# PaddlePaddle/Paddle

Hardware: AMD Instinct MI355X
Metric: tokens/sec (whole node) GPT-3-6.7B Fleet sharding-3 (higher is better)
Workload: dtype bf16; 1 GPU; model=gpt3-6.7b, global_batch=12, seq_len=2048, parallelism=sharding3_dp1

## Files before the change

### csrc/kernels/fa_bwd.hip

```cpp
#include "fa_common.h"

namespace pa {

template <int D>
__global__ void fa_bwd_delta_kernel(const short* __restrict__ dog, const short* __restrict__ og,
                                    float* __restrict__ delta, int H, int Sq,
                                    long long rows,
                                    long long do_sb, long long do_sh, long long do_ss,
                                    long long o_sb, long long o_sh, long long o_ss) {
  constexpr int LPR = D / 8, RPP = 256 / LPR, UNR = 4;
  const int sub = threadIdx.x % LPR;
  const int rin = threadIdx.x / LPR;
  const bool h_fast = do_sh < do_ss;
  for (long long r0 = (long long)blockIdx.x * (RPP * UNR); r0 < rows;
       r0 += (long long)gridDim.x * (RPP * UNR)) {
    shortx8 a[UNR], bb[UNR];
    long long di[UNR];
#pragma unroll
    for (int u = 0; u < UNR; ++u) {
      const long long r = r0 + u * RPP + rin;
      di[u] = -1;
      if (r < rows) {
        int sq, h, b;
        if (h_fast) {
// ... 200 lines not shown
      constexpr int elems = QB * D;
      for (int flat = tid * 8; flat < elems; flat += NT * 8) {
        int row = flat / D, col = flat % D;
        shortx8 qv, dv;
        if (q0 + row < Sq) {
          qv = *reinterpret_cast<const shortx8*>(qg + qbase + (long long)(q0 + row) * q_ss + col);
          dv = *reinterpret_cast<const shortx8*>(dog + dobase + (long long)(q0 + row) * do_ss + col);
        } else {
          for (int i = 0; i < 8; ++i) { qv[i] = 0; dv[i] = 0; }
        }
        const unsigned o = dkv_off<D>(row, col >> 3);
        *reinterpret_cast<shortx8*>(qbuf + o) = qv;
        *reinterpret_cast<shortx8*>(qbuf + TILE + o) = dv;
      }
    }
  };
  auto load_stats = [&](int q0, float* lse_o, float* delta_o) {
#pragma unroll
    for (int nt = 0; nt < 4; ++nt) {
      int q_abs = q0 + nt * 16 + l16;
      lse_o[nt] = (q_abs < Sq) ? lseg[lse_base + q_abs] : INFINITY;
      delta_o[nt] = (q_abs < Sq) ? deltag[lse_base + q_abs] : 0.f;
    }
  };

  char* const pw = lds + 4 * TILE + wq * PW;
  const unsigned lds_a = (unsigned)(size_t)(__attribute__((address_space(3))) char*)lds;
  const unsigned tr_q = l16 >> 2, tr_p = l16 & 3;
  unsigned bt_a[NDT];
#pragma unroll
  for (int dt = 0; dt < NDT; ++dt)
    bt_a[dt] = lds_a + dkv_off<D>(8 * lg + tr_q, 2 * dt + (tr_p >> 1)) + ((tr_p & 1) << 3);
  const unsigned pa_lo = lds_a + 4 * TILE + wq * PW + dkv_p_off(8 * lg + tr_q, tr_p);
  const unsigned pa_hi = lds_a + 4 * TILE + wq * PW + dkv_p_off(8 * lg + 4 + tr_q, tr_p);
  float lse_n[4], delta_n[4];
  if (q_start < Sq) {
    stage(q_start, lds);
    load_stats(q_start, lse_n, delta_n);
  }
  int cur = 0;
  for (int q0 = q_start; q0 < Sq; q0 += QB) {
    asm volatile("s_waitcnt vmcnt(0)" ::: "memory");
    __syncthreads();
    const unsigned boff = cur * (2 * TILE);
    const char* q_t = lds + boff;
    float lse_v[4], delta_v[4];
#pragma unroll
    for (int nt = 0; nt < 4; ++nt) { lse_v[nt] = lse_n[nt]; delta_v[nt] = delta_n[nt]; }
    if (q0 + QB < Sq) {
      stage(q0 + QB, lds + (cur ^ 1) * (2 * TILE));
      load_stats(q0 + QB, lse_n, delta_n);
    }
    cur ^= 1;
    const char* do_t = q_t + TILE;

    floatx4 pt[4];
    const int kv_abs0 = kv0 + wq * 16 + lg * 4;
#pragma unroll
    for (int nt = 0; nt < 4; ++nt) {
      floatx4 st = {0.f, 0.f, 0.f, 0.f};
#pragma unroll
      for (int kk = 0; kk < NKK; ++kk) {
        shortx8 qfr = *reinterpret_cast<const shortx8*>(
            q_t + dkv_off<D>(nt * 16 + l16, kk * 4 + lg));
        st = mfma_bf16(kf[kk], qfr, st);
      }
      const int q_abs = q0 + nt * 16 + l16;
      const bool bnd = (q0 + QB > Sq) || (kv0 + KVEXT > Skv) ||
                       (CAUSAL && q0 < kv0 + KVEXT);
      if (bnd) {
#pragma unroll
        for (int r = 0; r < 4; ++r) {
          int kv_abs = kv_abs0 + r;
          float p = __expf(st[r] * scale - lse_v[nt]);
          if (q_abs >= Sq || kv_abs >= Skv || (CAUSAL && kv_abs > q_abs)) p = 0.f;
          pt[nt][r] = p;
        }
      } else {
#pragma unroll
        for (int r = 0; r < 4; ++r)
          pt[nt][r] = __expf(st[r] * scale - lse_v[nt]);
      }
    }

    shortx8 pa[2];
    auto put_get = [&]() {
#pragma unroll
      for (int nt = 0; nt < 4; ++nt) {
        shortx4 v = {f2bf(pt[nt][0]), f2bf(pt[nt][1]), f2bf(pt[nt][2]), f2bf(pt[nt][3])};
        *reinterpret_cast<shortx4*>(pw + dkv_p_off(nt * 16 + l16, lg)) = v;
      }
      dkv_tr_read_pa(pa, pa_lo, pa_hi);
    };
    put_get();

    dkv_mma_tr<D, TILE>(dv_acc, pa[0], bt_a, boff);
    dkv_mma_tr<D, TILE + 32 * D * 2>(dv_acc, pa[1], bt_a, boff);

#pragma unroll
    for (int nt = 0; nt < 4; ++nt) {
      floatx4 dp = {0.f, 0.f, 0.f, 0.f};
#pragma unroll
      for (int kk = 0; kk < NKK; ++kk) {
        shortx8 bfr = *reinterpret_cast<const shortx8*>(
            do_t + dkv_off<D>(nt * 16 + l16, kk * 4 + lg));
        dp = mfma_bf16(vf[kk], bfr, dp);
      }
#pragma unroll
      for (int r = 0; r < 4; ++r)
        pt[nt][r] = pt[nt][r] * (dp[r] - delta_v[nt]) * scale;
    }
    put_get();

    dkv_mma_tr<D, 0>(dk_acc, pa[0], bt_a, boff);
    dkv_mma_tr<D, 32 * D * 2>(dk_acc, pa[1], bt_a, boff);
  }

#pragma unroll
  for (int r = 0; r < 4; ++r) {
    int row = kv0 + wq * 16 + lg * 4 + r;
    if (row >= Skv) continue;
#pragma unroll
    for (int dt = 0; dt < NDT; ++dt) {
      dkg[dkbase + (long long)row * dk_ss + dt * 16 + l16] = f2bf(dk_acc[dt][r]);
      dvg[dkbase + (long long)row * dk_ss + dt * 16 + l16] = f2bf(dv_acc[dt][r]);
    }
  }
}

template <int D, bool CAUSAL, bool MASKED, bool DROPOUT, bool VARLEN>
__launch_bounds__(256, 2)
__global__ void fa_bwd_dq32_kernel(const short* __restrict__ dog, const short* __restrict__ qg,
                                   const short* __restrict__ kg, const short* __restrict__ vg,
                                   const float* __restrict__ lseg, const float* __restrict__ deltag,
                                   short* __restrict__ dqg, int B, int H, int Sq, int Skv,
                                   float scale,
                                   long long q_sb, long long q_sh, long long q_ss,
                                   long long k_sb, long long k_sh, long long k_ss,
                                   long long do_sb, long long do_sh, long long do_ss,
                                   long long dq_sb, long long dq_sh, long long dq_ss,
                                   const short* __restrict__ maskg, long long m_sb,
                                   long long m_sh, long long m_sq,
                                   float pdrop, unsigned long long rseed,
                                   unsigned long long roffset,
                                   const int* __restrict__ cu_q,
                                   const int* __restrict__ cu_k,
                                   const int* __restrict__ bmap) {
  constexpr int NW = 4;
  constexpr int NT = NW * 64;
  constexpr int QB = NW * 32;
  constexpr int KB = 64;
  constexpr int NKS = D / 16;
  constexpr int NDT = D / 32;
  constexpr unsigned NAT_RS = D * 2;
  constexpr unsigned KT_RS = KB * 2;
  __shared__ char k_lds[KB * D * 2];
  __shared__ char v_lds[KB * D * 2];
  __shared__ char kt_lds[D * KB * 2];

  const int qblk = blockIdx.y;
  const int bh = blockIdx.x;
  int b = bh / H, h = bh % H;
  int q0, Sq_e = Sq, Skv_e = Skv, cdelta = 0, qglob0 = 0;
  long long qbase, dobase, dqbase, kvbase;
  if (VARLEN) {
    b = 0; h = bh;
    const int seq = bmap[2 * qblk];
    q0 = bmap[2 * qblk + 1];
    const int qs0 = cu_q[seq], ks0 = cu_k[seq];
    Sq_e = cu_q[seq + 1] - qs0;
    Skv_e = cu_k[seq + 1] - ks0;
    cdelta = Skv_e - Sq_e;
    qglob0 = qs0;
    qbase = (long long)qs0 * q_ss + (long long)h * q_sh;
    dobase = (long long)qs0 * do_ss + (long long)h * do_sh;
    dqbase = (long long)qs0 * dq_ss + (long long)h * dq_sh;
    kvbase = (long long)ks0 * k_ss + (long long)h * k_sh;
  } else {
    q0 = (CAUSAL ? ((int)gridDim.y - 1 - qblk) : qblk) * QB;
    qbase = (long long)b * q_sb + (long long)h * q_sh;
    dobase = (long long)b * do_sb + (long long)h * do_sh;
    dqbase = (long long)b * dq_sb + (long long)h * dq_sh;
    kvbase = (long long)b * k_sb + (long long)h * k_sh;
  }
  const long long lse_base = ((long long)bh) * Sq + qglob0;

  const int tid = threadIdx.x;
  const int lane = tid & 63;
  const int wq = tid >> 6;
  const int l32 = lane & 31;
  const int hi = lane >> 5;
  const int q0w = q0 + wq * 32;

  shortx8 qf[NKS], dof[NKS];
  {
    int row = q0w + l32;
    bool ok = row < Sq_e;
#pragma unroll
    for (int ks = 0; ks < NKS; ++ks) {
      if (ok) {
        shortx8 raw = *reinterpret_cast<const shortx8*>(
            qg + qbase + (long long)row * q_ss + ks * 16 + hi * 8);
#pragma unroll
        for (int i = 0; i < 8; ++i) qf[ks][i] = f2bf(bf2f(raw[i]) * scale);
        dof[ks] = *reinterpret_cast<const shortx8*>(
            dog + dobase + (long long)row * do_ss + ks * 16 + hi * 8);
      } else {
        for (int i = 0; i < 8; ++i) { qf[ks][i] = 0; dof[ks][i] = 0; }
      }
    }
  }
  const int q_abs = q0w + l32;
  const float lse_v = (q_abs < Sq_e) ? lseg[lse_base + q_abs] : 1e30f;
  const float delta_v = (q_abs < Sq_e) ? deltag[lse_base + q_abs] : 0.f;

  floatx16 dq_acc[NDT];
#pragma unroll
  for (int dt = 0; dt < NDT; ++dt)
#pragma unroll
    for (int r = 0; r < 16; ++r) dq_acc[dt][r] = 0.f;

  constexpr unsigned KSWZ = (D >= 128) ? 15u : 7u;
  int n_row[KB * D / (NT * 8)], n_colp[KB * D / (NT * 8)];
#pragma unroll
  for (int it = 0; it < KB * D / (NT * 8); ++it) {
    int flat = it * NT * 8 + tid * 8;
    int row = flat / D, col = flat % D;
    n_row[it] = row;
    n_colp[it] = col ^ ((row & (int)KSWZ) << 3);
  }

  const int kv_end = CAUSAL ? min(Skv_e, q0 + QB + cdelta) : Skv_e;
  for (int kv0 = 0; kv0 < kv_end; kv0 += KB) {
    if (kv0 + KB <= Skv_e) {
#pragma unroll
      for (int it = 0; it < KB * D / (NT * 8); ++it) {
        const short* ksrc = kg + kvbase + (long long)(kv0 + n_row[it]) * k_ss + n_colp[it];
        const short* vsrc = vg + kvbase + (long long)(kv0 + n_row[it]) * k_ss + n_colp[it];
        __builtin_amdgcn_global_load_lds(
            (const __attribute__((address_space(1))) unsigned int*)ksrc,
            (__attribute__((address_space(3))) unsigned int*)(k_lds + it * NT * 16 + (tid >> 6) * 64 * 16),
            16, 0, 0);
        __builtin_amdgcn_global_load_lds(
            (const __attribute__((address_space(1))) unsigned int*)vsrc,
            (__attribute__((address_space(3))) unsigned int*)(v_lds + it * NT * 16 + (tid >> 6) * 64 * 16),
            16, 0, 0);
      }
      const int rot = tid & 7;
      for (int flat = tid * 8; flat < KB * D; flat += NT * 8) {
        int row = flat / D, col = flat % D;
        shortx8 kv_ = *reinterpret_cast<const shortx8*>(
            kg + kvbase + (long long)(kv0 + row) * k_ss + col);
#pragma unroll
        for (int j = 0; j < 8; ++j) {
          int i = (j + rot) & 7;
          *reinterpret_cast<short*>(kt_lds + lds_off32(col + i, row * 2, KT_RS)) = kv_[i];
        }
      }
    } else {
      for (int flat = tid * 8; flat < KB * D; flat += NT * 8) {
        int row = flat / D, col = flat % D;
        shortx8 kv_, vv;
        if (kv0 + row < Skv_e) {
          kv_ = *reinterpret_cast<const shortx8*>(kg + kvbase + (long long)(kv0 + row) * k_ss + col);
          vv = *reinterpret_cast<const shortx8*>(vg + kvbase + (long long)(kv0 + row) * k_ss + col);
        } else {
          for (int i = 0; i < 8; ++i) { kv_[i] = 0; vv[i] = 0; }
        }
        *reinterpret_cast<shortx8*>(k_lds + lds_off32w(row, col * 2, NAT_RS, KSWZ)) = kv_;
        *reinterpret_cast<shortx8*>(v_lds + lds_off32w(row, col * 2, NAT_RS, KSWZ)) = vv;
        const int rot = tid & 7;
#pragma unroll
        for (int j = 0; j < 8; ++j) {
          int i = (j + rot) & 7;
          *reinterpret_cast<short*>(kt_lds + lds_off32(col + i, row * 2, KT_RS)) = kv_[i];
        }
      }
    }
    __syncthreads();

    floatx16 st[2], dp[2];
#pragma unroll
    for (int t = 0; t < 2; ++t) {
#pragma unroll
      for (int r = 0; r < 16; ++r) { st[t][r] = 0.f; dp[t][r] = 0.f; }
#pragma unroll
      for (int ks = 0; ks < NKS; ++ks) {
        shortx8 kf = *reinterpret_cast<const shortx8*>(
            k_lds + lds_off32w(t * 32 + l32, (ks * 16 + hi * 8) * 2, NAT_RS, KSWZ));
        st[t] = mfma32_bf16(kf, qf[ks], st[t]);
        shortx8 vf = *reinterpret_cast<const shortx8*>(
            v_lds + lds_off32w(t * 32 + l32, (ks * 16 + hi * 8) * 2, NAT_RS, KSWZ));
        dp[t] = mfma32_bf16(vf, dof[ks], dp[t]);
      }
    }

    if (MASKED && q_abs < Sq_e) {
      const short* mrow = maskg + (long long)b * m_sb + (long long)h * m_sh
                        + (long long)q_abs * m_sq;
#pragma unroll
      for (int t = 0; t < 2; ++t)
#pragma unroll
        for (int g = 0; g < 4; ++g) {
          long long kvb = kv0 + 32 * t + 8 * g + 4 * hi;
          if (kvb + 3 < Skv_e) {
            shortx4 mv = *reinterpret_cast<const shortx4*>(mrow + kvb);
#pragma unroll
            for (int j = 0; j < 4; ++j) st[t][4 * g + j] += bf2f(mv[j]);
          } else {
#pragma unroll
            for (int j = 0; j < 4; ++j)
              if (kvb + j < Skv_e) st[t][4 * g + j] += bf2f(mrow[kvb + j]);
          }
        }
    }
    const bool bnd = (kv0 + KB > Skv_e) || (CAUSAL && kv0 + KB > q_abs + cdelta);
    const float inv_keep = DROPOUT ? 1.f / (1.f - pdrop) : 1.f;
    const unsigned thr24 = DROPOUT ? (unsigned)(pdrop * 16777216.f) : 0u;
    const long long bh_ll = (long long)b * H + h;
#pragma unroll
    for (int t = 0; t < 2; ++t) {
      if (DROPOUT) {
#pragma unroll
        for (int g = 0; g < 4; ++g) {
          long long kvb = kv0 + 32 * t + 8 * g + 4 * hi;
          long long elem = (bh_ll * Sq + (q_abs + qglob0)) * (long long)Skv + kvb;
          uintx4 rv = philox10(rseed, roffset + (unsigned long long)(elem >> 2));
#pragma unroll
          for (int j = 0; j < 4; ++j)
            dp[t][4 * g + j] = ((rv[j] >> 8) >= thr24)
                                   ? dp[t][4 * g + j] * inv_keep : 0.f;
        }
      }
#pragma unroll
      for (int r = 0; r < 16; ++r) {
        float p = __expf(st[t][r] - lse_v);
        if (bnd) {
          int kv_abs = kv0 + 32 * t + (r & 3) + 8 * (r >> 2) + 4 * hi;
          if (kv_abs >= Skv_e || (CAUSAL && kv_abs > q_abs + cdelta)) p = 0.f;
        }
        st[t][r] = p * (dp[t][r] - delta_v) * scale;
      }
    }

#pragma unroll
    for (int ks = 0; ks < KB / 16; ++ks) {
      const int t = ks >> 1;
      const int kp = ks & 1;
      const int b0 = 8 * kp;
      int P0 = pack_bf2(st[t][b0 + 0], st[t][b0 + 1]);
      int P1 = pack_bf2(st[t][b0 + 2], st[t][b0 + 3]);
      int P2 = pack_bf2(st[t][b0 + 4], st[t][b0 + 5]);
      int P3 = pack_bf2(st[t][b0 + 6], st[t][b0 + 7]);
      int O1 = hi ? P2 : P0;
      int O2 = hi ? P3 : P1;
      int S1 = hi ? P0 : P2;
      int S2 = hi ? P1 : P3;
      intx2 ra = __builtin_amdgcn_permlane32_swap(S1, S2, false, false);
      intx2 rb = __builtin_amdgcn_permlane32_swap(S2, S1, false, false);
      int X1 = hi ? rb[0] : ra[1];
      int X2 = hi ? ra[0] : rb[1];
      intx4 paw;
      paw[0] = hi ? X1 : O1;
      paw[1] = hi ? X2 : O2;
      paw[2] = hi ? O1 : X1;
      paw[3] = hi ? O2 : X2;
      shortx8 pa = *reinterpret_cast<shortx8*>(&paw);
#pragma unroll
      for (int dt = 0; dt < NDT; ++dt) {
        shortx8 bf = *reinterpret_cast<const shortx8*>(
            kt_lds + lds_off32(dt * 32 + l32, (ks * 16 + hi * 8) * 2, KT_RS));
        dq_acc[dt] = mfma32_bf16(pa, bf, dq_acc[dt]);
      }
    }
    __syncthreads();
  }

#pragma unroll
  for (int r = 0; r < 16; ++r) {
    int rq = (r & 3) + 8 * (r >> 2) + 4 * hi;
    int row = q0w + rq;
    if (row >= Sq_e) continue;
#pragma unroll
    for (int dt = 0; dt < NDT; ++dt)
      dqg[dqbase + (long long)row * dq_ss + dt * 32 + l32] = f2bf(dq_acc[dt][r]);
  }
}

template <int D, bool CAUSAL, bool IS_DK, bool MASKED, bool DROPOUT, bool VARLEN>
__launch_bounds__(256, 2)
__global__ void fa_bwd_dkv32_kernel(const short* __restrict__ dog, const short* __restrict__ qg,
                                    const short* __restrict__ kg, const short* __restrict__ vg,
                                    const float* __restrict__ lseg, const float* __restrict__ deltag,
                                    short* __restrict__ outg,
                                    int B, int H, int Sq, int Skv, float scale,
                                    long long q_sb, long long q_sh, long long q_ss,
                                    long long k_sb, long long k_sh, long long k_ss,
                                    long long do_sb, long long do_sh, long long do_ss,
                                    long long dk_sb, long long dk_sh, long long dk_ss,
                                    const short* __restrict__ maskg, long long m_sb,
                                    long long m_sh, long long m_sq,
                                    float pdrop, unsigned long long rseed,
                                    unsigned long long roffset,
                                    const int* __restrict__ cu_q,
                                    const int* __restrict__ cu_k,
                                    const int* __restrict__ bmap) {
  constexpr int NW = 4;
  constexpr int NT = NW * 64;
  constexpr int KVB = NW * 32;
  constexpr int QT = 32;
  constexpr int NKS = D / 16;
  constexpr int NDT = D / 32;
  constexpr unsigned TR_RS = 64 * 2;
  __shared__ char t_lds[2][D * 64 * 2];
  __shared__ float stat_s[2][2 * QT];

  const int kvblk = blockIdx.y;
  const int bh = blockIdx.x;
  int b = bh / H, h = bh % H;
  int kv0, Sq_e = Sq, Skv_e = Skv, cdelta = 0, qglob0 = 0;
  long long qbase, dobase, kvbase, outbase;
  if (VARLEN) {
    b = 0; h = bh;
    const int seq = bmap[2 * kvblk];
    kv0 = bmap[2 * kvblk + 1];
    const int qs0 = cu_q[seq], ks0 = cu_k[seq];
    Sq_e = cu_q[seq + 1] - qs0;
    Skv_e = cu_k[seq + 1] - ks0;
    cdelta = Skv_e - Sq_e;
    qglob0 = qs0;
    qbase = (long long)qs0 * q_ss + (long long)h * q_sh;
    dobase = (long long)qs0 * do_ss + (long long)h * do_sh;
    kvbase = (long long)ks0 * k_ss + (long long)h * k_sh;
    outbase = (long long)ks0 * dk_ss + (long long)h * dk_sh;
  } else {
    kv0 = kvblk * KVB;
    qbase = (long long)b * q_sb + (long long)h * q_sh;
    dobase = (long long)b * do_sb + (long long)h * do_sh;
    kvbase = (long long)b * k_sb + (long long)h * k_sh;
    outbase = (long long)b * dk_sb + (long long)h * dk_sh;
  }
  const long long lse_base = ((long long)bh) * Sq + qglob0;

  const int tid = threadIdx.x;
  const int lane = tid & 63;
  const int wq = tid >> 6;
  const int l32 = lane & 31;
  const int hi = lane >> 5;
  const int kv0w = kv0 + wq * 32;
  const int kv_lane = kv0w + l32;

  shortx8 kf[NKS], vf[IS_DK ? NKS : 1];
  {
    bool ok = kv_lane < Skv_e;
#pragma unroll
    for (int ks = 0; ks < NKS; ++ks) {
      if (ok) {
        kf[ks] = *reinterpret_cast<const shortx8*>(
            kg + kvbase + (long long)kv_lane * k_ss + ks * 16 + hi * 8);
        if (IS_DK)
          vf[ks] = *reinterpret_cast<const shortx8*>(
              vg + kvbase + (long long)kv_lane * k_ss + ks * 16 + hi * 8);
      } else {
        for (int i = 0; i < 8; ++i) { kf[ks][i] = 0; if (IS_DK) vf[ks][i] = 0; }
      }
    }
  }

  floatx16 acc[NDT];
#pragma unroll
  for (int dt = 0; dt < NDT; ++dt)
#pragma unroll
    for (int r = 0; r < 16; ++r) acc[dt][r] = 0.f;

  auto stage = [&](int buf, int q0) {
    if (tid < QT) {
      int qa = q0 + tid;
      stat_s[buf][tid] = (qa < Sq_e) ? lseg[lse_base + qa] : 1e30f;
      if (IS_DK)
        stat_s[buf][QT + tid] = (qa < Sq_e) ? deltag[lse_base + qa] : 0.f;
    }
    const int rot = tid & 7;
    for (int flat = tid * 8; flat < QT * D; flat += NT * 8) {
      int row = flat / D, col = flat % D;
      shortx8 v;
      if (q0 + row < Sq_e) {
        const short* src = IS_DK
            ? qg + qbase + (long long)(q0 + row) * q_ss + col
            : dog + dobase + (long long)(q0 + row) * do_ss + col;
        v = *reinterpret_cast<const shortx8*>(src);
      } else {
        for (int i = 0; i < 8; ++i) v[i] = 0;
      }
#pragma unroll
      for (int j = 0; j < 8; ++j) {
        int i = (j + rot) & 7;
        *reinterpret_cast<short*>(t_lds[buf] + lds_off32(col + i, row * 2, TR_RS)) = v[i];
      }
    }
  };

  const int q_start = CAUSAL ? (max(0, kv0 - cdelta) / QT) * QT : 0;
  stage(0, q_start);
  __syncthreads();
  int cur = 0;
  for (int q0 = q_start; q0 < Sq_e; q0 += QT) {
    if (q0 + QT < Sq_e) stage(cur ^ 1, q0 + QT);

    const int q_lane = q0 + l32;
    const bool qok = q_lane < Sq_e;
    floatx16 st, dp;
#pragma unroll
    for (int r = 0; r < 16; ++r) { st[r] = 0.f; dp[r] = 0.f; }
#pragma unroll
    for (int ks = 0; ks < NKS; ++ks) {
      shortx8 qa;
      if (qok)
        qa = *reinterpret_cast<const shortx8*>(
            qg + qbase + (long long)q_lane * q_ss + ks * 16 + hi * 8);
      else
        for (int i = 0; i < 8; ++i) qa[i] = 0;
      st = mfma32_bf16(qa, kf[ks], st);
      if (IS_DK) {
        shortx8 da;
        if (qok)
          da = *reinterpret_cast<const shortx8*>(
              dog + dobase + (long long)q_lane * do_ss + ks * 16 + hi * 8);
        else
// ... 128 lines not shown
```

### csrc/kernels/fa_common.h

```cpp
#pragma once
#include <type_traits>

#include "common.h"
#include "api.h"

namespace pa {

typedef __attribute__((ext_vector_type(16))) float floatx16;
typedef __attribute__((ext_vector_type(2))) int intx2;

__device__ __forceinline__ floatx16 mfma32_bf16(shortx8 a, shortx8 b, floatx16 c) {
  return __builtin_amdgcn_mfma_f32_32x32x16_bf16(a, b, c, 0, 0, 0);
}

__device__ __forceinline__ unsigned lds_off32(unsigned row, unsigned col_bytes,
                                              unsigned row_stride) {
  return row * row_stride + (col_bytes ^ ((row & 7u) << 4));
}

__device__ __forceinline__ unsigned lds_off32w(unsigned row, unsigned col_bytes,
                                               unsigned row_stride, unsigned mask) {
  return row * row_stride + (col_bytes ^ ((row & mask) << 4));
}

__device__ __forceinline__ int pack_bf2(float a, float b) {
  unsigned lo = (unsigned short)f2bf(a);
  unsigned hi = (unsigned short)f2bf(b);
  return (int)(lo | (hi << 16));
}

struct FaBlock {
  int b, h, r0, Sq_e, Skv_e, cdelta, q_tok0, k_tok0;
};

template <bool VARLEN>
__device__ __forceinline__ FaBlock fa_block(const FaArgs& a, const int* bmap,
                                            int dense_r0) {
  FaBlock g;
  const int bh = blockIdx.x, blk = blockIdx.y;
  if (VARLEN) {
    const int seq = bmap[2 * blk];
    g.b = 0; g.h = bh;
    g.r0 = bmap[2 * blk + 1];
    g.q_tok0 = a.cu_q[seq];
    g.k_tok0 = a.cu_k[seq];
    g.Sq_e = a.cu_q[seq + 1] - g.q_tok0;
    g.Skv_e = a.cu_k[seq + 1] - g.k_tok0;
    g.cdelta = g.Skv_e - g.Sq_e;
  } else {
    g.b = bh / a.h; g.h = bh % a.h;
    g.r0 = dense_r0;
    g.q_tok0 = 0; g.k_tok0 = 0;
    g.Sq_e = a.sq; g.Skv_e = a.skv;
    g.cdelta = 0;
  }
  return g;
}

__device__ __forceinline__ long long fa_base(const FaBlock& g, const FaStride& s,
                                             int head, int tok0) {
  return (long long)g.b * s.b + (long long)head * s.h + (long long)tok0 * s.s;
}

template <class F>
inline void fa_bool(bool v, F&& f) {
  if (v) f(std::true_type{}); else f(std::false_type{});
}

template <class F>
inline void fa_dispatch(const FaArgs& a, F&& f) {
  fa_bool(a.dh == 128, [&](auto d128) {
    fa_bool(a.causal, [&](auto c) {
      fa_bool(a.mask != nullptr, [&](auto m) {
        fa_bool(a.pdrop > 0.f, [&](auto p) {
          f(std::integral_constant<int, decltype(d128)::value ? 128 : 64>{}, c, m, p);
        });
      });
    });
  });
}

}
```

### csrc/kernels/fa_fwd32.hip

```cpp
#include "fa_common.h"

namespace pa {

template <int D, bool CAUSAL, bool MASKED, bool DROPOUT, bool VARLEN>
__launch_bounds__(256, 2)
__global__ void fa_fwd32_kernel(const FaArgs a) {
  const short* __restrict__ qg = (const short*)a.q;
  const short* __restrict__ kg = (const short*)a.k;
  const short* __restrict__ vg = (const short*)a.v;
  short* __restrict__ og = (short*)a.o;
  float* __restrict__ lseg = a.lse;
  const int H = a.h, Sq = a.sq, Skv = a.skv;
  const float scale = a.scale;
  const long long q_ss = a.q_s.s, k_ss = a.k_s.s, o_ss = a.o_s.s;
  const short* __restrict__ maskg = (const short*)a.mask;
  const long long m_sb = a.m_s.b, m_sh = a.m_s.h, m_sq = a.m_s.s;
  const float pdrop = a.pdrop;
  const unsigned long long rseed = a.seed, roffset = a.offset;
  constexpr int NW = 4;
  constexpr int NT = NW * 64;
  constexpr int QB = NW * 32;
  constexpr int KB = 64;
  constexpr int NKS = D / 16;
  constexpr int NDT = D / 32;
  constexpr unsigned K_RS = D * 2;
  constexpr unsigned VT_RS = KB * 2;
  __shared__ char k_lds[2][KB * D * 2];
  __shared__ char vt_lds[2][D * KB * 2];

  const FaBlock g = fa_block<VARLEN>(
      a, a.q_bmap, (CAUSAL ? (int)(gridDim.y - 1 - blockIdx.y) : (int)blockIdx.y) * QB);
  const int b = g.b, h = g.h, q0 = g.r0, Sq_e = g.Sq_e, Skv_e = g.Skv_e;
  const int cdelta = g.cdelta, qglob0 = g.q_tok0;
  const long long qbase = fa_base(g, a.q_s, h, g.q_tok0);
  const long long kbase = fa_base(g, a.k_s, h / (H / a.hkv), g.k_tok0);
  const long long obase = fa_base(g, a.o_s, h, g.q_tok0);

  const int tid = threadIdx.x;
  const int lane = tid & 63;
  const int wq = tid >> 6;
  const int l32 = lane & 31;
  const int hi = lane >> 5;
  const int q0w = q0 + wq * 32;

  shortx8 qf[NKS];
  {
    int row = q0w + l32;
    bool ok = row < Sq_e;
#pragma unroll
    for (int ks = 0; ks < NKS; ++ks) {
      if (ok) {
        shortx8 raw = *reinterpret_cast<const shortx8*>(
            qg + qbase + (long long)row * q_ss + ks * 16 + hi * 8);
#pragma unroll
        for (int i = 0; i < 8; ++i) qf[ks][i] = f2bf(bf2f(raw[i]) * scale);
      } else {
        for (int i = 0; i < 8; ++i) qf[ks][i] = 0;
      }
    }
  }

  floatx16 oacc[NDT];
#pragma unroll
  for (int dt = 0; dt < NDT; ++dt)
#pragma unroll
    for (int r = 0; r < 16; ++r) oacc[dt][r] = 0.f;
  float m_run = -INFINITY, l_run = 0.f;

  const int kv_end = CAUSAL ? min(Skv_e, q0 + QB + cdelta) : Skv_e;

  constexpr unsigned KSWZ = (D >= 128) ? 15u : 7u;
  int k_row[KB * D / (NT * 8)], k_colp[KB * D / (NT * 8)];
#pragma unroll
  for (int it = 0; it < KB * D / (NT * 8); ++it) {
    int flat = it * NT * 8 + tid * 8;
    int row = flat / D, col = flat % D;
    k_row[it] = row;
    k_colp[it] = col ^ ((row & (int)KSWZ) << 3);
  }

  auto stage = [&](int buf, int kv0) {
    if (kv0 + KB <= Skv_e) {
#pragma unroll
      for (int it = 0; it < KB * D / (NT * 8); ++it) {
        const short* src = kg + kbase + (long long)(kv0 + k_row[it]) * k_ss + k_colp[it];
        char* dst = k_lds[buf] + it * NT * 16 + (tid >> 6) * 64 * 16;
        __builtin_amdgcn_global_load_lds(
            (const __attribute__((address_space(1))) unsigned int*)src,
            (__attribute__((address_space(3))) unsigned int*)dst, 16, 0, 0);
      }
    } else {
      for (int flat = tid * 8; flat < KB * D; flat += NT * 8) {
        int row = flat / D, col = flat % D;
        shortx8 val;
        if (kv0 + row < Skv_e)
          val = *reinterpret_cast<const shortx8*>(kg + kbase + (long long)(kv0 + row) * k_ss + col);
        else
          for (int i = 0; i < 8; ++i) val[i] = 0;
        *reinterpret_cast<shortx8*>(k_lds[buf] + lds_off32w(row, col * 2, K_RS, KSWZ)) = val;
      }
    }
    {
      const int rot = tid & 7;
      for (int flat = tid * 8; flat < KB * D; flat += NT * 8) {
        int row = flat / D, col = flat % D;
        shortx8 val;
        if (kv0 + row < Skv_e)
          val = *reinterpret_cast<const shortx8*>(vg + kbase + (long long)(kv0 + row) * k_ss + col);
        else
          for (int i = 0; i < 8; ++i) val[i] = 0;
#pragma unroll
        for (int j = 0; j < 8; ++j) {
          int i = (j + rot) & 7;
          *reinterpret_cast<short*>(vt_lds[buf] + lds_off32(col + i, row * 2, VT_RS)) = val[i];
        }
      }
    }
  };

  stage(0, 0);
  __syncthreads();
  int cur = 0;
  for (int kv0 = 0; kv0 < kv_end; kv0 += KB) {
    if (kv0 + KB < kv_end) stage(cur ^ 1, kv0 + KB);

    floatx16 st[2];
#pragma unroll
    for (int t = 0; t < 2; ++t) {
#pragma unroll
      for (int r = 0; r < 16; ++r) st[t][r] = 0.f;
#pragma unroll
      for (int ks = 0; ks < NKS; ++ks) {
        shortx8 kf = *reinterpret_cast<const shortx8*>(
            k_lds[cur] + lds_off32w(t * 32 + l32, (ks * 16 + hi * 8) * 2, K_RS, KSWZ));
        st[t] = mfma32_bf16(kf, qf[ks], st[t]);
      }
    }

    const int q_abs = q0w + l32;
    if (MASKED && q_abs < Sq_e) {
      const short* mrow = maskg + (long long)b * m_sb + (long long)h * m_sh
                        + (long long)q_abs * m_sq;
#pragma unroll
      for (int t = 0; t < 2; ++t)
#pragma unroll
        for (int g = 0; g < 4; ++g) {
          long long kvb = kv0 + 32 * t + 8 * g + 4 * hi;
          if (kvb + 3 < Skv_e) {
            shortx4 mv = *reinterpret_cast<const shortx4*>(mrow + kvb);
#pragma unroll
            for (int j = 0; j < 4; ++j) st[t][4 * g + j] += bf2f(mv[j]);
          } else {
#pragma unroll
            for (int j = 0; j < 4; ++j)
              if (kvb + j < Skv_e) st[t][4 * g + j] += bf2f(mrow[kvb + j]);
          }
        }
    }
    float mx = -INFINITY;
    const bool boundary = (kv0 + KB > Skv_e) || (CAUSAL && kv0 + KB > q_abs + cdelta);
    if (boundary) {
#pragma unroll
      for (int t = 0; t < 2; ++t)
#pragma unroll
        for (int r = 0; r < 16; ++r) {
          int kv_abs = kv0 + 32 * t + (r & 3) + 8 * (r >> 2) + 4 * hi;
          float v = st[t][r];
          if (kv_abs >= Skv_e || (CAUSAL && kv_abs > q_abs + cdelta)) v = -INFINITY;
          st[t][r] = v;
          mx = fmaxf(mx, v);
        }
    } else {
#pragma unroll
      for (int t = 0; t < 2; ++t)
#pragma unroll
        for (int r = 0; r < 16; ++r) {
          mx = fmaxf(mx, st[t][r]);
        }
    }
    mx = fmaxf(mx, __shfl_xor(mx, 32, 64));
    const float THR = 8.f;
    const bool grow = (mx > m_run + THR) || (m_run == -INFINITY);
    float m_new = grow ? fmaxf(m_run, mx) : m_run;
    float corr = (m_run == -INFINITY) ? 0.f : __expf(m_run - m_new);
    if (__any(grow && m_run != -INFINITY)) {
      l_run *= corr;
#pragma unroll
      for (int dt = 0; dt < NDT; ++dt)
#pragma unroll
        for (int r = 0; r < 16; ++r) {
          int rq = (r & 3) + 8 * (r >> 2) + 4 * hi;
          float c = __shfl(corr, rq, 64);
          oacc[dt][r] *= c;
        }
    }
    m_run = m_new;
    float psum = 0.f;
#pragma unroll
    for (int t = 0; t < 2; ++t)
#pragma unroll
      for (int r = 0; r < 16; ++r) {
        float p = (st[t][r] == -INFINITY) ? 0.f : __expf(st[t][r] - m_run);
        st[t][r] = p;
        psum += p;
      }
    psum += __shfl_xor(psum, 32, 64);
    l_run += psum;
    if (DROPOUT) {
      const float inv_keep = 1.f / (1.f - pdrop);
      const unsigned thr24 = (unsigned)(pdrop * 16777216.f);
      const long long bh_ll = (long long)b * H + h;
#pragma unroll
      for (int t = 0; t < 2; ++t)
#pragma unroll
        for (int g = 0; g < 4; ++g) {
          long long kvb = kv0 + 32 * t + 8 * g + 4 * hi;
          long long elem = (bh_ll * Sq + (q_abs + qglob0)) * (long long)Skv + kvb;
          uintx4 rv = philox10(rseed, roffset + (unsigned long long)(elem >> 2));
#pragma unroll
          for (int j = 0; j < 4; ++j)
            st[t][4 * g + j] = ((rv[j] >> 8) >= thr24)
                                   ? st[t][4 * g + j] * inv_keep : 0.f;
        }
    }

#pragma unroll
    for (int ks = 0; ks < KB / 16; ++ks) {
      const int t = ks >> 1;
      const int kp = ks & 1;
      const int b0 = 8 * kp;
      int P0 = pack_bf2(st[t][b0 + 0], st[t][b0 + 1]);
      int P1 = pack_bf2(st[t][b0 + 2], st[t][b0 + 3]);
      int P2 = pack_bf2(st[t][b0 + 4], st[t][b0 + 5]);
      int P3 = pack_bf2(st[t][b0 + 6], st[t][b0 + 7]);
      int O1 = hi ? P2 : P0;
      int O2 = hi ? P3 : P1;
      int S1 = hi ? P0 : P2;
      int S2 = hi ? P1 : P3;
      intx2 ra = __builtin_amdgcn_permlane32_swap(S1, S2, false, false);
      intx2 rb = __builtin_amdgcn_permlane32_swap(S2, S1, false, false);
      int X1 = hi ? rb[0] : ra[1];
      int X2 = hi ? ra[0] : rb[1];
      intx4 paw;
      paw[0] = hi ? X1 : O1;
      paw[1] = hi ? X2 : O2;
      paw[2] = hi ? O1 : X1;
      paw[3] = hi ? O2 : X2;
      shortx8 pa = *reinterpret_cast<shortx8*>(&paw);
#pragma unroll
      for (int dt = 0; dt < NDT; ++dt) {
        shortx8 vf = *reinterpret_cast<const shortx8*>(
            vt_lds[cur] + lds_off32(dt * 32 + l32, (ks * 16 + hi * 8) * 2, VT_RS));
        oacc[dt] = mfma32_bf16(pa, vf, oacc[dt]);
      }
    }
    __syncthreads();
    cur ^= 1;
  }

  float inv_l = (l_run > 0.f) ? 1.f / l_run : 0.f;
#pragma unroll
  for (int r = 0; r < 16; ++r) {
    int rq = (r & 3) + 8 * (r >> 2) + 4 * hi;
    float il = __shfl(inv_l, rq, 64);
    int row = q0w + rq;
    if (row >= Sq_e) continue;
#pragma unroll
    for (int dt = 0; dt < NDT; ++dt)
      og[obase + (long long)row * o_ss + dt * 32 + l32] = f2bf(oacc[dt][r] * il);
  }
  if (hi == 0 && q0w + l32 < Sq_e)
    lseg[(long long)(b * H + h) * Sq + qglob0 + q0w + l32] =
        (l_run > 0.f) ? m_run + __logf(l_run) : -INFINITY;
}

void flash_attn_fwd(const FaArgs& a, hipStream_t s) {
  const bool varlen = a.cu_q != nullptr;
  const dim3 grid((unsigned)(a.b * a.h),
                  (unsigned)(varlen ? a.n_qblocks : cdiv(a.sq, 128)));
  fa_dispatch(a, [&](auto D, auto C, auto M, auto P) {
    if (!varlen)
      hipLaunchKernelGGL((fa_fwd32_kernel<D(), C(), M(), P(), false>), grid, dim3(256), 0, s, a);
    else if constexpr (!M())
      hipLaunchKernelGGL((fa_fwd32_kernel<D(), C(), false, P(), true>), grid, dim3(256), 0, s, a);
  });
}

__global__ void fa_dropout_mask_kernel(unsigned char* __restrict__ out,
                                       float p, unsigned long long seed,
                                       unsigned long long offset,
                                       long long total) {
  long long i4 = (long long)blockIdx.x * blockDim.x + threadIdx.x;
  long long base = i4 * 4;
  if (base >= total) return;
  unsigned thr24 = (unsigned)(p * 16777216.f);
  uintx4 rv = philox10(seed, offset + (unsigned long long)i4);
#pragma unroll
  for (int j = 0; j < 4; ++j)
    if (base + j < total) out[base + j] = ((rv[j] >> 8) >= thr24) ? 1 : 0;
}

void fa_dropout_mask(void* out, int64_t total, float p, uint64_t seed,
                     uint64_t offset, hipStream_t s) {
  long long n4 = (total + 3) / 4;
  dim3 g((unsigned)hmin<long long>((n4 + 255) / 256, 1 << 30));
  hipLaunchKernelGGL(fa_dropout_mask_kernel, g, dim3(256), 0, s,
                     (unsigned char*)out, p, seed, offset, total);
}

}
```

Measured before the change: 25020 tokens/s.

## Use ds_read_b64_tr_b16 transposed LDS reads instead of materialized K/V transposes

Drops the separately transposed K and V LDS copies, which were built with scalar 2-byte LDS writes, in both the flash-attention forward kernel and the dQ backward kernel. The P·V and P·K products now read the natural-layout tiles through the gfx950 ds_read_b64_tr_b16 transpose-load instruction, using a new shared swizzle so both layouts stay conflict-light. The dQ kernel also gains double-buffered async global->LDS staging of K and V, and the forward path now loads V asynchronously as well. This trades larger LDS usage (four tiles) and inline asm with explicit waitcnts for fewer LDS stores and more overlap of loads with compute.

```diff
diff --git a/csrc/kernels/fa_bwd.hip b/csrc/kernels/fa_bwd.hip
--- a/csrc/kernels/fa_bwd.hip
+++ b/csrc/kernels/fa_bwd.hip
@@ -376,11 +376,8 @@
   constexpr int KB = 64;
   constexpr int NKS = D / 16;
   constexpr int NDT = D / 32;
-  constexpr unsigned NAT_RS = D * 2;
-  constexpr unsigned KT_RS = KB * 2;
-  __shared__ char k_lds[KB * D * 2];
-  __shared__ char v_lds[KB * D * 2];
-  __shared__ char kt_lds[D * KB * 2];
+  constexpr int TILE = KB * D * 2;
+  __shared__ __attribute__((aligned(16))) char lds[4 * TILE];
 
   const int qblk = blockIdx.y;
   const int bh = blockIdx.x;
@@ -444,64 +441,26 @@
 #pragma unroll
     for (int r = 0; r < 16; ++r) dq_acc[dt][r] = 0.f;
 
-  constexpr unsigned KSWZ = (D >= 128) ? 15u : 7u;
-  int n_row[KB * D / (NT * 8)], n_colp[KB * D / (NT * 8)];
-#pragma unroll
-  for (int it = 0; it < KB * D / (NT * 8); ++it) {
-    int flat = it * NT * 8 + tid * 8;
-    int row = flat / D, col = flat % D;
-    n_row[it] = row;
-    n_colp[it] = col ^ ((row & (int)KSWZ) << 3);
+  const unsigned lds_a = (unsigned)(size_t)(__attribute__((address_space(3))) char*)lds;
+  unsigned tr_a[2][NDT];
+#pragma unroll
+  for (int dt = 0; dt < NDT; ++dt) {
+    tr_a[0][dt] = fa_tr_addr<D>(lds_a, lane, dt, 0);
+    tr_a[1][dt] = fa_tr_addr<D>(lds_a, lane, dt, 16);
   }
 
   const int kv_end = CAUSAL ? min(Skv_e, q0 + QB + cdelta) : Skv_e;
+  if (kv_end > 0) fa_stage_kv<D, NT>(lds, kg, vg, kvbase, k_ss, 0, Skv_e, tid);
+  int cur = 0;
   for (int kv0 = 0; kv0 < kv_end; kv0 += KB) {
-    if (kv0 + KB <= Skv_e) {
-#pragma unroll
-      for (int it = 0; it < KB * D / (NT * 8); ++it) {
-        const short* ksrc = kg + kvbase + (long long)(kv0 + n_row[it]) * k_ss + n_colp[it];
-        const short* vsrc = vg + kvbase + (long long)(kv0 + n_row[it]) * k_ss + n_colp[it];
-        __builtin_amdgcn_global_load_lds(
-            (const __attribute__((address_space(1))) unsigned int*)ksrc,
-            (__attribute__((address_space(3))) unsigned int*)(k_lds + it * NT * 16 + (tid >> 6) * 64 * 16),
-            16, 0, 0);
-        __builtin_amdgcn_global_load_lds(
-            (const __attribute__((address_space(1))) unsigned int*)vsrc,
-            (__attribute__((address_space(3))) unsigned int*)(v_lds + it * NT * 16 + (tid >> 6) * 64 * 16),
-            16, 0, 0);
-      }
-      const int rot = tid & 7;
-      for (int flat = tid * 8; flat < KB * D; flat += NT * 8) {
-        int row = flat / D, col = flat % D;
-        shortx8 kv_ = *reinterpret_cast<const shortx8*>(
-            kg + kvbase + (long long)(kv0 + row) * k_ss + col);
-#pragma unroll
-        for (int j = 0; j < 8; ++j) {
-          int i = (j + rot) & 7;
-          *reinterpret_cast<short*>(kt_lds + lds_off32(col + i, row * 2, KT_RS)) = kv_[i];
-        }
-      }
-    } else {
-      for (int flat = tid * 8; flat < KB * D; flat += NT * 8) {
-        int row = flat / D, col = flat % D;
-        shortx8 kv_, vv;
-        if (kv0 + row < Skv_e) {
-          kv_ = *reinterpret_cast<const shortx8*>(kg + kvbase + (long long)(kv0 + row) * k_ss + col);
-          vv = *reinterpret_cast<const shortx8*>(vg + kvbase + (long long)(kv0 + row) * k_ss + col);
-        } else {
-          for (int i = 0; i < 8; ++i) { kv_[i] = 0; vv[i] = 0; }
-        }
-        *reinterpret_cast<shortx8*>(k_lds + lds_off32w(row, col * 2, NAT_RS, KSWZ)) = kv_;
-        *reinterpret_cast<shortx8*>(v_lds + lds_off32w(row, col * 2, NAT_RS, KSWZ)) = vv;
-        const int rot = tid & 7;
-#pragma unroll
-        for (int j = 0; j < 8; ++j) {
-          int i = (j + rot) & 7;
-          *reinterpret_cast<short*>(kt_lds + lds_off32(col + i, row * 2, KT_RS)) = kv_[i];
-        }
-      }
-    }
+    asm volatile("s_waitcnt vmcnt(0)" ::: "memory");
     __syncthreads();
+    const unsigned boff = cur * (2 * TILE);
+    const char* k_t = lds + boff;
+    const char* v_t = k_t + TILE;
+    if (kv0 + KB < kv_end)
+      fa_stage_kv<D, NT>(lds + (cur ^ 1) * (2 * TILE), kg, vg, kvbase, k_ss, kv0 + KB, Skv_e, tid);
+    cur ^= 1;
 
     floatx16 st[2], dp[2];
 #pragma unroll
@@ -511,10 +470,10 @@
 #pragma unroll
       for (int ks = 0; ks < NKS; ++ks) {
         shortx8 kf = *reinterpret_cast<const shortx8*>(
-            k_lds + lds_off32w(t * 32 + l32, (ks * 16 + hi * 8) * 2, NAT_RS, KSWZ));
+            k_t + fa_kv_off<D>(t * 32 + l32, ks * 2 + hi));
         st[t] = mfma32_bf16(kf, qf[ks], st[t]);
         shortx8 vf = *reinterpret_cast<const shortx8*>(
-            v_lds + lds_off32w(t * 32 + l32, (ks * 16 + hi * 8) * 2, NAT_RS, KSWZ));
+            v_t + fa_kv_off<D>(t * 32 + l32, ks * 2 + hi));
         dp[t] = mfma32_bf16(vf, dof[ks], dp[t]);
       }
     }
@@ -567,11 +526,11 @@
       }
     }
 
-#pragma unroll
-    for (int ks = 0; ks < KB / 16; ++ks) {
-      const int t = ks >> 1;
-      const int kp = ks & 1;
-      const int b0 = 8 * kp;
+    auto dq_step = [&](auto KS) {
+      constexpr int ks = decltype(KS)::value;
+      constexpr int t = ks >> 1;
+      constexpr int kp = ks & 1;
+      constexpr int b0 = 8 * kp;
       int P0 = pack_bf2(st[t][b0 + 0], st[t][b0 + 1]);
       int P1 = pack_bf2(st[t][b0 + 2], st[t][b0 + 3]);
       int P2 = pack_bf2(st[t][b0 + 4], st[t][b0 + 5]);
@@ -590,14 +549,18 @@
       paw[2] = hi ? O1 : X1;
       paw[3] = hi ? O2 : X2;
       shortx8 pa = *reinterpret_cast<shortx8*>(&paw);
-#pragma unroll
-      for (int dt = 0; dt < NDT; ++dt) {
-        shortx8 bf = *reinterpret_cast<const shortx8*>(
-            kt_lds + lds_off32(dt * 32 + l32, (ks * 16 + hi * 8) * 2, KT_RS));
-        dq_acc[dt] = mfma32_bf16(pa, bf, dq_acc[dt]);
-      }
-    }
-    __syncthreads();
+      shortx8 bf[NDT];
+      unsigned ka[NDT];
+#pragma unroll
+      for (int dt = 0; dt < NDT; ++dt) ka[dt] = boff + tr_a[kp][dt];
+      fa_tr_read<D, ks * 16 * D * 2>(bf, ka);
+#pragma unroll
+      for (int dt = 0; dt < NDT; ++dt) dq_acc[dt] = mfma32_bf16(pa, bf[dt], dq_acc[dt]);
+    };
+    dq_step(std::integral_constant<int, 0>{});
+    dq_step(std::integral_constant<int, 1>{});
+    dq_step(std::integral_constant<int, 2>{});
+    dq_step(std::integral_constant<int, 3>{});
   }
 
 #pragma unroll
diff --git a/csrc/kernels/fa_common.h b/csrc/kernels/fa_common.h
--- a/csrc/kernels/fa_common.h
+++ b/csrc/kernels/fa_common.h
@@ -18,9 +18,101 @@
   return row * row_stride + (col_bytes ^ ((row & 7u) << 4));
 }
 
-__device__ __forceinline__ unsigned lds_off32w(unsigned row, unsigned col_bytes,
-                                               unsigned row_stride, unsigned mask) {
-  return row * row_stride + (col_bytes ^ ((row & mask) << 4));
+template <int D>
+__device__ __forceinline__ unsigned fa_kv_swz(unsigned row) {
+  if constexpr (D == 128)
+    return ((row & 3u) << 2) | ((row >> 3) & 3u);
+  else
+    return (((row >> 1) & 1u) << 2) | ((row >> 3) & 3u);
+}
+
+template <int D>
+__device__ __forceinline__ unsigned fa_kv_off(unsigned row, unsigned ch) {
+  return row * (D * 2) + ((ch ^ fa_kv_swz<D>(row)) << 4);
+}
+
+template <int D, int NT>
+__device__ __forceinline__ void fa_stage_kv(char* buf, const short* __restrict__ kg,
+                                            const short* __restrict__ vg, long long base,
+                                            long long k_ss, int kv0, int Skv_e, int tid) {
+  constexpr int KB = 64;
+  constexpr int TILE = KB * D * 2;
+  if (kv0 + KB <= Skv_e) {
+#pragma unroll
+    for (int it = 0; it < KB * D / (NT * 8); ++it) {
+      const int flat = it * NT * 8 + tid * 8;
+      const int row = flat / D, col = flat % D;
+      const long long src = base + (long long)(kv0 + row) * k_ss
+                          + (col ^ (int)(fa_kv_swz<D>(row) << 3));
+      char* dst = buf + it * NT * 16 + (tid >> 6) * 64 * 16;
+      __builtin_amdgcn_global_load_lds(
+          (const __attribute__((address_space(1))) unsigned int*)(kg + src),
+          (__attribute__((address_space(3))) unsigned int*)dst, 16, 0, 0);
+      __builtin_amdgcn_global_load_lds(
+          (const __attribute__((address_space(1))) unsigned int*)(vg + src),
+          (__attribute__((address_space(3))) unsigned int*)(dst + TILE), 16, 0, 0);
+    }
+  } else {
+    for (int flat = tid * 8; flat < KB * D; flat += NT * 8) {
+      const int row = flat / D, col = flat % D;
+      shortx8 kv_, vv;
+      if (kv0 + row < Skv_e) {
+        kv_ = *reinterpret_cast<const shortx8*>(kg + base + (long long)(kv0 + row) * k_ss + col);
+        vv = *reinterpret_cast<const shortx8*>(vg + base + (long long)(kv0 + row) * k_ss + col);
+      } else {
+        for (int i = 0; i < 8; ++i) { kv_[i] = 0; vv[i] = 0; }
+      }
+      const unsigned o = fa_kv_off<D>(row, col >> 3);
+      *reinterpret_cast<shortx8*>(buf + o) = kv_;
+      *reinterpret_cast<shortx8*>(buf + TILE + o) = vv;
+    }
+  }
+}
+
+template <int D>
+__device__ __forceinline__ unsigned fa_tr_addr(unsigned img, int lane, int dt, int r0) {
+  const unsigned g = lane >> 4, q = (lane >> 2) & 3u, p = lane & 3u;
+  return img + fa_kv_off<D>(r0 + 8 * (g >> 1) + q, 4 * dt + 2 * (g & 1u) + (p >> 1))
+       + ((p & 1u) << 3) - r0 * (D * 2);
+}
+
+template <int D, int LO>
+__device__ __forceinline__ void fa_tr_read(shortx8 (&b)[D / 32], const unsigned (&a)[D / 32]) {
+  constexpr int HI = LO + 4 * D * 2;
+  static_assert(HI < 65536, "ds offset field");
+  if constexpr (D == 128) {
+    shortx4 l0, h0, l1, h1, l2, h2, l3, h3;
+    asm volatile(
+        "ds_read_b64_tr_b16 %0, %8 offset:%12\n\t"
+        "ds_read_b64_tr_b16 %1, %8 offset:%13\n\t"
+        "ds_read_b64_tr_b16 %2, %9 offset:%12\n\t"
+        "ds_read_b64_tr_b16 %3, %9 offset:%13\n\t"
+        "ds_read_b64_tr_b16 %4, %10 offset:%12\n\t"
+        "ds_read_b64_tr_b16 %5, %10 offset:%13\n\t"
+        "ds_read_b64_tr_b16 %6, %11 offset:%12\n\t"
+        "ds_read_b64_tr_b16 %7, %11 offset:%13\n\t"
+        "s_waitcnt lgkmcnt(0)"
+        : "=&v"(l0), "=&v"(h0), "=&v"(l1), "=&v"(h1), "=&v"(l2), "=&v"(h2), "=&v"(l3), "=&v"(h3)
+        : "v"(a[0]), "v"(a[1]), "v"(a[2]), "v"(a[3]), "n"(LO), "n"(HI)
+        : "memory");
+    b[0] = __builtin_shufflevector(l0, h0, 0, 1, 2, 3, 4, 5, 6, 7);
+    b[1] = __builtin_shufflevector(l1, h1, 0, 1, 2, 3, 4, 5, 6, 7);
+    b[2] = __builtin_shufflevector(l2, h2, 0, 1, 2, 3, 4, 5, 6, 7);
+    b[3] = __builtin_shufflevector(l3, h3, 0, 1, 2, 3, 4, 5, 6, 7);
+  } else {
+    shortx4 l0, h0, l1, h1;
+    asm volatile(
+        "ds_read_b64_tr_b16 %0, %4 offset:%6\n\t"
+        "ds_read_b64_tr_b16 %1, %4 offset:%7\n\t"
+        "ds_read_b64_tr_b16 %2, %5 offset:%6\n\t"
+        "ds_read_b64_tr_b16 %3, %5 offset:%7\n\t"
+        "s_waitcnt lgkmcnt(0)"
+        : "=&v"(l0), "=&v"(h0), "=&v"(l1), "=&v"(h1)
+        : "v"(a[0]), "v"(a[1]), "n"(LO), "n"(HI)
+        : "memory");
+    b[0] = __builtin_shufflevector(l0, h0, 0, 1, 2, 3, 4, 5, 6, 7);
+    b[1] = __builtin_shufflevector(l1, h1, 0, 1, 2, 3, 4, 5, 6, 7);
+  }
 }
 
 __device__ __forceinline__ int pack_bf2(float a, float b) {
diff --git a/csrc/kernels/fa_fwd32.hip b/csrc/kernels/fa_fwd32.hip
--- a/csrc/kernels/fa_fwd32.hip
+++ b/csrc/kernels/fa_fwd32.hip
@@ -23,10 +23,8 @@
   constexpr int KB = 64;
   constexpr int NKS = D / 16;
   constexpr int NDT = D / 32;
-  constexpr unsigned K_RS = D * 2;
-  constexpr unsigned VT_RS = KB * 2;
-  __shared__ char k_lds[2][KB * D * 2];
-  __shared__ char vt_lds[2][D * KB * 2];
+  constexpr int TILE = KB * D * 2;
+  __shared__ __attribute__((aligned(16))) char lds[4 * TILE];
 
   const FaBlock g = fa_block<VARLEN>(
       a, a.q_bmap, (CAUSAL ? (int)(gridDim.y - 1 - blockIdx.y) : (int)blockIdx.y) * QB);
@@ -69,60 +67,24 @@
 
   const int kv_end = CAUSAL ? min(Skv_e, q0 + QB + cdelta) : Skv_e;
 
-  constexpr unsigned KSWZ = (D >= 128) ? 15u : 7u;
-  int k_row[KB * D / (NT * 8)], k_colp[KB * D / (NT * 8)];
-#pragma unroll
-  for (int it = 0; it < KB * D / (NT * 8); ++it) {
-    int flat = it * NT * 8 + tid * 8;
-    int row = flat / D, col = flat % D;
-    k_row[it] = row;
-    k_colp[it] = col ^ ((row & (int)KSWZ) << 3);
-  }
-
-  auto stage = [&](int buf, int kv0) {
-    if (kv0 + KB <= Skv_e) {
-#pragma unroll
-      for (int it = 0; it < KB * D / (NT * 8); ++it) {
-        const short* src = kg + kbase + (long long)(kv0 + k_row[it]) * k_ss + k_colp[it];
-        char* dst = k_lds[buf] + it * NT * 16 + (tid >> 6) * 64 * 16;
-        __builtin_amdgcn_global_load_lds(
-            (const __attribute__((address_space(1))) unsigned int*)src,
-            (__attribute__((address_space(3))) unsigned int*)dst, 16, 0, 0);
-      }
-    } else {
-      for (int flat = tid * 8; flat < KB * D; flat += NT * 8) {
-        int row = flat / D, col = flat % D;
-        shortx8 val;
-        if (kv0 + row < Skv_e)
-          val = *reinterpret_cast<const shortx8*>(kg + kbase + (long long)(kv0 + row) * k_ss + col);
-        else
-          for (int i = 0; i < 8; ++i) val[i] = 0;
-        *reinterpret_cast<shortx8*>(k_lds[buf] + lds_off32w(row, col * 2, K_RS, KSWZ)) = val;
-      }
-    }
-    {
-      const int rot = tid & 7;
-      for (int flat = tid * 8; flat < KB * D; flat += NT * 8) {
-        int row = flat / D, col = flat % D;
-        shortx8 val;
-        if (kv0 + row < Skv_e)
-          val = *reinterpret_cast<const shortx8*>(vg + kbase + (long long)(kv0 + row) * k_ss + col);
-        else
-          for (int i = 0; i < 8; ++i) val[i] = 0;
-#pragma unroll
-        for (int j = 0; j < 8; ++j) {
-          int i = (j + rot) & 7;
-          *reinterpret_cast<short*>(vt_lds[buf] + lds_off32(col + i, row * 2, VT_RS)) = val[i];
-        }
-      }
-    }
-  };
-
-  stage(0, 0);
-  __syncthreads();
+  const unsigned lds_a = (unsigned)(size_t)(__attribute__((address_space(3))) char*)lds;
+  unsigned tr_a[2][NDT];
+#pragma unroll
+  for (int dt = 0; dt < NDT; ++dt) {
+    tr_a[0][dt] = fa_tr_addr<D>(lds_a, lane, dt, 0);
+    tr_a[1][dt] = fa_tr_addr<D>(lds_a, lane, dt, 16);
+  }
+
+  if (kv_end > 0) fa_stage_kv<D, NT>(lds, kg, vg, kbase, k_ss, 0, Skv_e, tid);
   int cur = 0;
   for (int kv0 = 0; kv0 < kv_end; kv0 += KB) {
-    if (kv0 + KB < kv_end) stage(cur ^ 1, kv0 + KB);
+    asm volatile("s_waitcnt vmcnt(0)" ::: "memory");
+    __syncthreads();
+    const unsigned boff = cur * (2 * TILE);
+    const char* k_t = lds + boff;
+    if (kv0 + KB < kv_end)
+      fa_stage_kv<D, NT>(lds + (cur ^ 1) * (2 * TILE), kg, vg, kbase, k_ss, kv0 + KB, Skv_e, tid);
+    cur ^= 1;
 
     floatx16 st[2];
 #pragma unroll
@@ -132,7 +94,7 @@
 #pragma unroll
       for (int ks = 0; ks < NKS; ++ks) {
         shortx8 kf = *reinterpret_cast<const shortx8*>(
-            k_lds[cur] + lds_off32w(t * 32 + l32, (ks * 16 + hi * 8) * 2, K_RS, KSWZ));
+            k_t + fa_kv_off<D>(t * 32 + l32, ks * 2 + hi));
         st[t] = mfma32_bf16(kf, qf[ks], st[t]);
       }
     }
@@ -224,10 +186,10 @@
         }
     }
 
-#pragma unroll
-    for (int ks = 0; ks < KB / 16; ++ks) {
-      const int t = ks >> 1;
-      const int kp = ks & 1;
+    auto pv_step = [&](auto KS) {
+      constexpr int ks = decltype(KS)::value;
+      constexpr int t = ks >> 1;
+      constexpr int kp = ks & 1;
       const int b0 = 8 * kp;
       int P0 = pack_bf2(st[t][b0 + 0], st[t][b0 + 1]);
       int P1 = pack_bf2(st[t][b0 + 2], st[t][b0 + 3]);
@@ -247,15 +209,18 @@
       paw[2] = hi ? O1 : X1;
       paw[3] = hi ? O2 : X2;
       shortx8 pa = *reinterpret_cast<shortx8*>(&paw);
-#pragma unroll
-      for (int dt = 0; dt < NDT; ++dt) {
-        shortx8 vf = *reinterpret_cast<const shortx8*>(
-            vt_lds[cur] + lds_off32(dt * 32 + l32, (ks * 16 + hi * 8) * 2, VT_RS));
-        oacc[dt] = mfma32_bf16(pa, vf, oacc[dt]);
-      }
-    }
-    __syncthreads();
-    cur ^= 1;
+      shortx8 vf[NDT];
+      unsigned va[NDT];
+#pragma unroll
+      for (int dt = 0; dt < NDT; ++dt) va[dt] = boff + tr_a[kp][dt];
+      fa_tr_read<D, TILE + ks * 16 * D * 2>(vf, va);
+#pragma unroll
+      for (int dt = 0; dt < NDT; ++dt) oacc[dt] = mfma32_bf16(pa, vf[dt], oacc[dt]);
+    };
+    pv_step(std::integral_constant<int, 0>{});
+    pv_step(std::integral_constant<int, 1>{});
+    pv_step(std::integral_constant<int, 2>{});
+    pv_step(std::integral_constant<int, 3>{});
   }
 
   float inv_l = (l_run > 0.f) ? 1.f / l_run : 0.f;
```

After: 26100 tokens/s (median of 6 runs). 4.3% higher.
